# UBC-AWP/vision-sam3-yolo-lameless

Hardware: AMD Instinct MI355X
Metric: frames/sec (whole node) for YOLO+SAM3+DINOv3 feature extraction, 1080p clips (higher is better)
Workload: dtype f16; 1 GPU; BASELINE cfg#5, dense schedule: fused per-frame path on a synthetic 5 s @ 30 fps 1080p clip (150 unique BGR frames resident in HBM): YOLOv8-l detect (letterbox 384x640, NMS, scale_boxes; f16 plan) -> SAM (Hiera-B+ image encoder + FPN at 1024x1024, box-prompted mask decoder, 1080p mask + statistics + contour features) + DINOv3 ViT-L/16 embed (224x224) on EVERY frame; per-frame records packed, gathe; parallelism=one clip per GPU, 1 GPU(s), one gather per step, streams=7

## Files before the change

### vision-sam3-yolo-lameless_amd/csrc/nms.hip

```cpp
#include "common.h"

namespace {

constexpr int MAX_A = 16384;

__global__ __launch_bounds__(256) void nms_filter_kernel(const float* __restrict__ pred, int n, int A, int nc,
                                                         float conf, unsigned long long* __restrict__ keys,
                                                         int* __restrict__ counts) {
  const int64_t total = (int64_t)n * A;
  const int row_len = 4 + nc;
  for (int64_t i = (int64_t)blockIdx.x * blockDim.x + threadIdx.x; i < total; i += (int64_t)gridDim.x * blockDim.x) {
    const int img = (int)(i / A);
    const int a = (int)(i - (int64_t)img * A);
    const float* row = pred + i * row_len + 4;
    float best = row[0];
    for (int c = 1; c < nc; ++c) {
      const float v = row[c];
      best = v > best ? v : best;
    }
    if (best > conf) {
      const int slot = atomicAdd(&counts[img], 1);
      const unsigned long long key =
          ((unsigned long long)__float_as_uint(best) << 32) | (unsigned long long)(0xFFFFFFFFu - (unsigned)a);
      keys[(int64_t)img * A + slot] = key;
    }
  }
}

struct Box {
  float x1, y1, x2, y2, area;
};

__device__ __forceinline__ bool iou_gt(const Box& a, const Box& b, double thr) {
  const float xx1 = a.x1 > b.x1 ? a.x1 : b.x1;
  const float yy1 = a.y1 > b.y1 ? a.y1 : b.y1;
  const float xx2 = a.x2 < b.x2 ? a.x2 : b.x2;
  const float yy2 = a.y2 < b.y2 ? a.y2 : b.y2;
  float w = xx2 - xx1;
  w = w > 0.f ? w : 0.f;
  float h = yy2 - yy1;
  h = h > 0.f ? h : 0.f;
  const float inter = w * h;
  const float ovr = inter / (a.area + b.area - inter);
  return (double)ovr > thr;
}

__device__ __forceinline__ void bitonic_sort_desc(unsigned long long* keys, int npow2) {
  const int tid = threadIdx.x;
  for (int k = 2; k <= npow2; k <<= 1) {
    for (int j = k >> 1; j > 0; j >>= 1) {
      for (int i = tid; i < npow2; i += 1024) {
        const int ixj = i ^ j;
        if (ixj > i) {
          const unsigned long long a = keys[i], b = keys[ixj];
          const bool desc = (i & k) == 0;
          if (desc ? (a < b) : (a > b)) {
            keys[i] = b;
            keys[ixj] = a;
          }
        }
      }
      __syncthreads();
    }
  }
}

template <class Emit>
__device__ __forceinline__ int greedy_blocks(const float* __restrict__ SB, int count, double iou, int max_keep, unsigned char* supp,
                                             Box* kept, Emit emit) {
  __shared__ int s_nk;
  __shared__ int s_total;
  __shared__ int s_kept_idx[64];
  const int tid = threadIdx.x;
  const int lane = tid & 63;
  if (tid == 0) s_total = 0;
  __syncthreads();
  const int nblk = (count + 63) / 64;
// ... 159 lines not shown
  int mine = 0;
  for (int i = tid; i < npow2; i += 1024) {
    const bool v = i < n && (valid == nullptr || valid[i] != 0);
    keys[i] = v ? (((unsigned long long)score_order_key(scores[i]) << 32) | (unsigned long long)(0xFFFFFFFFu - (unsigned)i)) : 0ull;
    supp[i] = 0;
    mine += v ? 1 : 0;
    if (i < n) keep_out[i] = -1;
  }
#pragma unroll
  for (int o = 32; o > 0; o >>= 1) mine += __shfl_xor(mine, o, 64);
  if ((tid & 63) == 0 && mine) atomicAdd(&s_count, mine);
  __syncthreads();
  const int count = s_count;
  bitonic_sort_desc(keys, npow2);

  for (int i = tid; i < count; i += 1024) {
    const unsigned a = 0xFFFFFFFFu - (unsigned)(keys[i] & 0xFFFFFFFFull);
    const float* r = boxes + (int64_t)a * ldb;
    sbox[i * 5 + 0] = r[0];
    sbox[i * 5 + 1] = r[1];
    sbox[i * 5 + 2] = r[2];
    sbox[i * 5 + 3] = r[3];
    sbox[i * 5 + 4] = (r[2] - r[0]) * (r[3] - r[1]);
  }
  __syncthreads();

  const int total = greedy_blocks(sbox, count, iou, count, supp, kept, [&](int, int i, int o) {
    keep_out[o] = (int)(0xFFFFFFFFu - (unsigned)(keys[i] & 0xFFFFFFFFull));
  });
  if (tid == 0) count_out[0] = total;
}

}

extern "C" int64_t lmx_nms_workspace_bytes(int n, int A) {
  if (n <= 0 || A <= 0) return 0;
  return 256 + ((int64_t)n * 4 + 255) / 256 * 256 + (int64_t)n * A * 8 + (int64_t)n * A * 5 * 4;
}

extern "C" int lmx_k_nms(const float* pred, int n, int A, int nc, float conf, double iou, int max_det, float max_wh,
                         float* boxes, float* scores, int32_t* cls, int32_t* src, int32_t* counts, void* workspace,
                         lmx_stream_t stream) {
  LMX_REQUIRE(pred && boxes && scores && cls && src && counts && workspace, "lmx_k_nms: null pointer");
  LMX_REQUIRE(n > 0 && A > 0 && A <= MAX_A && nc > 0 && max_det > 0, "lmx_k_nms: n=%d A=%d (<=%d) nc=%d max_det=%d", n,
              A, MAX_A, nc, max_det);
  LMX_REQUIRE((((uintptr_t)workspace) & 255) == 0, "lmx_k_nms: workspace must be 256-byte aligned");
  hipStream_t st = reinterpret_cast<hipStream_t>(stream);
  char* ws = reinterpret_cast<char*>(workspace);
  int* cand_counts = reinterpret_cast<int*>(ws);
  const int64_t cnt_bytes = ((int64_t)n * 4 + 255) / 256 * 256;
  unsigned long long* keys = reinterpret_cast<unsigned long long*>(ws + cnt_bytes);
  float* sbox = reinterpret_cast<float*>(ws + cnt_bytes + (int64_t)n * A * 8);
  LMX_HIP(hipMemsetAsync(cand_counts, 0, (size_t)n * 4, st));
  int64_t g = ((int64_t)n * A + 255) / 256;
  if (g > 2048) g = 2048;
  hipLaunchKernelGGL(nms_filter_kernel, dim3((unsigned)g), dim3(256), 0, st, pred, n, A, nc, conf, keys, cand_counts);
  int rc = lmx_launch_check("nms_filter_kernel");
  if (rc) return rc;
  int npow2 = 64;
  while (npow2 < A) npow2 <<= 1;
  const size_t smem = (size_t)npow2 * 9 + 64 * sizeof(Box);
  int dev;
  LMX_TRY(lmx_stream_device(st, &dev));
  LMX_TRY(lmx_allow_lds(reinterpret_cast<const void*>(&nms_greedy_kernel), (int)((size_t)MAX_A * 9 + 64 * sizeof(Box)), dev));
  hipLaunchKernelGGL(nms_greedy_kernel, dim3(n), dim3(1024), smem, st, pred, A, nc, iou, max_det, max_wh, keys, cand_counts,
                     sbox, boxes, scores, cls, src, counts);
  return lmx_launch_check("nms_greedy_kernel");
}

extern "C" int lmx_k_nms_boxes(const float* boxes, int64_t ldb, const float* scores, const uint8_t* valid, int n, double iou,
                               int32_t* keep_out, int32_t* count_out, void* workspace, lmx_stream_t stream) {
  LMX_REQUIRE(boxes && scores && keep_out && count_out && workspace, "lmx_k_nms_boxes: null pointer");
  LMX_REQUIRE(n > 0 && n <= MAX_A && ldb >= 4, "lmx_k_nms_boxes: n=%d (1..%d) ldb=%lld", n, MAX_A, (long long)ldb);
  LMX_REQUIRE((((uintptr_t)workspace) & 15) == 0, "lmx_k_nms_boxes: workspace must be 16-byte aligned");
  int npow2 = 64;
  while (npow2 < n) npow2 <<= 1;
  const size_t smem = (size_t)npow2 * 9 + 64 * sizeof(Box);
  hipStream_t st = reinterpret_cast<hipStream_t>(stream);
  int dev;
  LMX_TRY(lmx_stream_device(st, &dev));
  LMX_TRY(lmx_allow_lds(reinterpret_cast<const void*>(&nms_boxes_kernel), (int)((size_t)MAX_A * 9 + 64 * sizeof(Box)), dev));
  hipLaunchKernelGGL(nms_boxes_kernel, dim3(1), dim3(1024), smem, st, boxes, ldb, scores, valid, n, iou, reinterpret_cast<float*>(workspace),
                     keep_out, count_out);
  return lmx_launch_check("nms_boxes_kernel");
}
```

### vision-sam3-yolo-lameless_amd/csrc/pre.hip

```cpp
#include "common.h"

namespace {

constexpr int PRECISION_BITS = 32 - 8 - 2;

__device__ __forceinline__ uint8_t clip8(int v) {
  v >>= PRECISION_BITS;
  return (uint8_t)(v < 0 ? 0 : (v > 255 ? 255 : v));
}

constexpr int RESIZE_H_MAX_ROW = 16384;
__global__ __launch_bounds__(256) void pil_resize_h_kernel(const uint8_t* __restrict__ src, uint8_t* __restrict__ dst,
                                                           int n, int sh, int sw, int dw,
                                                           const int32_t* __restrict__ bounds,
                                                           const int32_t* __restrict__ kk, int ksize, int swap_rb) {
  __shared__ __attribute__((aligned(16))) uint8_t rowbuf[RESIZE_H_MAX_ROW];
  const int rowb = sw * 3;
  for (int64_t row = blockIdx.x; row < (int64_t)n * sh; row += gridDim.x) {
    const uint8_t* srow = src + row * rowb;
    const int mis = (int)(reinterpret_cast<uintptr_t>(srow) & 15);
    const int head = mis ? 16 - mis : 0;
    for (int i = threadIdx.x; i < head && i < rowb; i += blockDim.x) rowbuf[i] = srow[i];
    const int nvec = (rowb - head) > 0 ? (rowb - head) / 16 : 0;
    for (int v = threadIdx.x; v < nvec; v += blockDim.x) {
      const u32x4 x = *reinterpret_cast<const u32x4*>(srow + head + v * 16);
      uint8_t* d = rowbuf + head + v * 16;
      if ((head & 3) == 0) {
        reinterpret_cast<unsigned*>(d)[0] = x[0];
        reinterpret_cast<unsigned*>(d)[1] = x[1];
        reinterpret_cast<unsigned*>(d)[2] = x[2];
        reinterpret_cast<unsigned*>(d)[3] = x[3];
      } else {
#pragma unroll
        for (int e = 0; e < 16; ++e) d[e] = (uint8_t)(x[e >> 2] >> (8 * (e & 3)));
      }
    }
    for (int i = head + nvec * 16 + threadIdx.x; i < rowb; i += blockDim.x) rowbuf[i] = srow[i];
    __syncthreads();
    uint8_t* drow = dst + row * dw * 3;
    for (int xo = threadIdx.x; xo < dw; xo += blockDim.x) {
      const int xmin = bounds[2 * xo], cnt = bounds[2 * xo + 1];
      const int32_t* k = kk + (int64_t)xo * ksize;
      const uint8_t* s = rowbuf + xmin * 3;
      int a0 = 1 << (PRECISION_BITS - 1), a1 = a0, a2 = a0;
      for (int x = 0; x < cnt; ++x) {
        const int c = k[x];
        a0 += (int)s[3 * x + 0] * c;
        a1 += (int)s[3 * x + 1] * c;
        a2 += (int)s[3 * x + 2] * c;
      }
      uint8_t* d = drow + xo * 3;
      if (swap_rb) {
        d[0] = clip8(a2);
        d[1] = clip8(a1);
        d[2] = clip8(a0);
      } else {
        d[0] = clip8(a0);
        d[1] = clip8(a1);
        d[2] = clip8(a2);
      }
    }
    __syncthreads();
  }
}

__global__ __launch_bounds__(256) void pil_resize_v_kernel(const uint8_t* __restrict__ src, uint8_t* __restrict__ dst,
                                                           int n, int sh, int dh, int w,
                                                           const int32_t* __restrict__ bounds,
                                                           const int32_t* __restrict__ kk, int ksize) {
  const int rowb = w * 3;
  const int64_t total = (int64_t)n * dh * rowb;
  for (int64_t i = (int64_t)blockIdx.x * blockDim.x + threadIdx.x; i < total; i += (int64_t)gridDim.x * blockDim.x) {
    const int xb = (int)(i % rowb);
    const int64_t r = i / rowb;
    const int yo = (int)(r % dh);
    const int img = (int)(r / dh);
    const int ymin = bounds[2 * yo], cnt = bounds[2 * yo + 1];
    const int32_t* k = kk + (int64_t)yo * ksize;
    const uint8_t* s = src + ((int64_t)img * sh + ymin) * rowb + xb;
    int a = 1 << (PRECISION_BITS - 1);
    for (int y = 0; y < cnt; ++y) a += (int)s[(int64_t)y * rowb] * k[y];
    dst[i] = clip8(a);
  }
}

__global__ __launch_bounds__(256) void pil_resize_v4_kernel(const uint8_t* __restrict__ src, uint8_t* __restrict__ dst, int n, int sh,
                                                            int dh, int w, const int32_t* __restrict__ bounds,
                                                            const int32_t* __restrict__ kk, int ksize) {
  const int rowb = w * 3, roww = rowb / 4;
  const int64_t total = (int64_t)n * dh * roww;
  for (int64_t i = (int64_t)blockIdx.x * blockDim.x + threadIdx.x; i < total; i += (int64_t)gridDim.x * blockDim.x) {
    const int xw = (int)(i % roww);
    const int64_t r = i / roww;
    const int yo = (int)(r % dh);
    const int img = (int)(r / dh);
    const int ymin = bounds[2 * yo], cnt = bounds[2 * yo + 1];
    const int32_t* k = kk + (int64_t)yo * ksize;
    const uint8_t* s = src + ((int64_t)img * sh + ymin) * rowb + xw * 4;
    int a0 = 1 << (PRECISION_BITS - 1), a1 = a0, a2 = a0, a3 = a0;
    for (int y = 0; y < cnt; ++y) {
      const unsigned v = *reinterpret_cast<const unsigned*>(s + (int64_t)y * rowb);
      const int c = k[y];
      a0 += (int)(v & 255u) * c;
      a1 += (int)((v >> 8) & 255u) * c;
      a2 += (int)((v >> 16) & 255u) * c;
      a3 += (int)(v >> 24) * c;
    }
    *reinterpret_cast<unsigned*>(dst + r * rowb + xw * 4) =
        (unsigned)clip8(a0) | ((unsigned)clip8(a1) << 8) | ((unsigned)clip8(a2) << 16) | ((unsigned)clip8(a3) << 24);
  }
}

__global__ __launch_bounds__(256) void patchify_norm_kernel(const uint8_t* __restrict__ img, half_t* __restrict__ out,
                                                            int n, int ih, int iw, int top, int left, int gh, int gw,
                                                            int P, int64_t ldo, const float* __restrict__ lut) {
  const int ch = gh * P, cw = gw * P;
  const int64_t total = (int64_t)n * ch * cw;
  for (int64_t i = (int64_t)blockIdx.x * blockDim.x + threadIdx.x; i < total; i += (int64_t)gridDim.x * blockDim.x) {
    const int x = (int)(i % cw);
    const int64_t r = i / cw;
    const int y = (int)(r % ch);
    const int b = (int)(r / ch);
    const uint8_t* s = img + (((int64_t)b * ih + top + y) * iw + left + x) * 3;
    const int py = y / P, ky = y - py * P, px = x / P, kx = x - px * P;
    half_t* d = out + (((int64_t)b * gh + py) * gw + px) * ldo + (ky * P + kx) * 3;
#pragma unroll
    for (int c = 0; c < 3; ++c) d[c] = (half_t)lut[c * 256 + s[c]];
  }
}

constexpr int FR_ROWS = 8;
constexpr int FR_COLS = 256;
constexpr int FR_MAX_LDS = 65536;

__global__ __launch_bounds__(FR_COLS) void float_resize_patchify_kernel(
    const uint8_t* __restrict__ src, half_t* __restrict__ out, int sh, int sw, int gh, int gw, int P, int64_t ldo,
    const int32_t* __restrict__ bh, const float* __restrict__ kh, int ksh, const int32_t* __restrict__ bv,
    const float* __restrict__ kv, int ksv, int seg_cols, float rescale, float m0, float m1, float m2, float s0, float s1,
    float s2, int swap_rb) {
  extern __shared__ __attribute__((aligned(16))) float seg[];
  const int tid = threadIdx.x;
  const int dh = gh * P, dw = gw * P;
  const int img = blockIdx.z;
  const int x0 = blockIdx.x * FR_COLS, xo = x0 + tid;
  const int y0 = blockIdx.y * FR_ROWS;
  const bool live = xo < dw;
  const int xl = (x0 + FR_COLS < dw ? x0 + FR_COLS : dw) - 1;
  int c_lo = bh[2 * x0];
  c_lo = c_lo < 0 ? 0 : (c_lo > sw ? sw : c_lo);
  int c_hi = bh[2 * xl] + bh[2 * xl + 1];
  c_hi = c_hi > sw ? sw : c_hi;
  if (c_hi > c_lo + seg_cols) c_hi = c_lo + seg_cols;
  if (c_hi < c_lo) c_hi = c_lo;
  int xmin = 0, xcnt = 0;
  if (live) {
    xmin = bh[2 * xo];
    xcnt = bh[2 * xo + 1];
    if (xmin < c_lo) xmin = c_lo;
    if (xcnt > ksh) xcnt = ksh;
    if (xcnt > c_hi - xmin) xcnt = c_hi - xmin;
    if (xcnt < 0) xcnt = 0;
  }
// ... 44 lines not shown
        f[3] = (float)(x[q] >> 24) * rescale;
        d[q] = f;
      }
    }
    for (int i = head + nvec * 16 + tid; i < nbytes; i += FR_COLS) s[i] = (float)srow[i] * rescale;
    __syncthreads();
    float h0 = 0.f, h1 = 0.f, h2 = 0.f;
    const float* p = s + (xmin - c_lo) * 3;
    for (int j = 0; j < xcnt; ++j) {
      const float w = kx[j];
      h0 = __builtin_fmaf(p[3 * j + 0], w, h0);
      h1 = __builtin_fmaf(p[3 * j + 1], w, h1);
      h2 = __builtin_fmaf(p[3 * j + 2], w, h2);
    }
#pragma unroll
    for (int r = 0; r < FR_ROWS; ++r) {
      if (y >= ymin[r] && y < ymin[r] + ycnt[r]) {
        const float w = kv[(int64_t)(y0 + r) * ksv + (y - ymin[r])];
        acc[r][0] = __builtin_fmaf(h0, w, acc[r][0]);
        acc[r][1] = __builtin_fmaf(h1, w, acc[r][1]);
        acc[r][2] = __builtin_fmaf(h2, w, acc[r][2]);
      }
    }
    __syncthreads();
  }
  if (!live) return;
  const int px = xo / P, kxp = xo - px * P;
#pragma unroll
  for (int r = 0; r < FR_ROWS; ++r) {
    const int yo = y0 + r;
    if (yo >= dh) break;
    const int py = yo / P, ky = yo - py * P;
    half_t* d = out + (((int64_t)img * gh + py) * gw + px) * ldo + (ky * P + kxp) * 3;
    d[0] = (half_t)(((swap_rb ? acc[r][2] : acc[r][0]) - m0) / s0);
    d[1] = (half_t)((acc[r][1] - m1) / s1);
    d[2] = (half_t)(((swap_rb ? acc[r][0] : acc[r][2]) - m2) / s2);
  }
}

inline int grid_for(int64_t total) {
  int64_t g = (total + 255) / 256;
  if (g > 256 * 8) g = 256 * 8;
  if (g < 1) g = 1;
  return (int)g;
}

}

extern "C" int lmx_k_pil_resize_h(const uint8_t* src, uint8_t* dst, int n, int sh, int sw, int dw, const int32_t* bounds,
                                  const int32_t* kk, int ksize, int swap_rb, lmx_stream_t stream) {
  LMX_REQUIRE(src && dst && bounds && kk, "lmx_k_pil_resize_h: null pointer");
  LMX_REQUIRE(n > 0 && sh > 0 && sw > 0 && dw > 0 && ksize > 0, "lmx_k_pil_resize_h: shape");
  LMX_REQUIRE(sw * 3 <= RESIZE_H_MAX_ROW, "lmx_k_pil_resize_h: source rows wider than %d pixels are not staged", RESIZE_H_MAX_ROW / 3);
  int64_t rows = (int64_t)n * sh;
  hipLaunchKernelGGL(pil_resize_h_kernel, dim3((unsigned)(rows < 256 * 16 ? rows : 256 * 16)), dim3(256), 0,
                     reinterpret_cast<hipStream_t>(stream), src, dst, n, sh, sw, dw, bounds, kk, ksize, swap_rb);
  return lmx_launch_check("pil_resize_h_kernel");
}

extern "C" int lmx_k_pil_resize_v(const uint8_t* src, uint8_t* dst, int n, int sh, int dh, int w, const int32_t* bounds,
                                  const int32_t* kk, int ksize, lmx_stream_t stream) {
  LMX_REQUIRE(src && dst && bounds && kk, "lmx_k_pil_resize_v: null pointer");
  LMX_REQUIRE(n > 0 && sh > 0 && dh > 0 && w > 0 && ksize > 0, "lmx_k_pil_resize_v: shape");
  if ((w * 3) % 4 == 0 && (((uintptr_t)src | (uintptr_t)dst) & 3) == 0) {
    hipLaunchKernelGGL(pil_resize_v4_kernel, dim3(grid_for((int64_t)n * dh * (w * 3 / 4))), dim3(256), 0,
                       reinterpret_cast<hipStream_t>(stream), src, dst, n, sh, dh, w, bounds, kk, ksize);
    return lmx_launch_check("pil_resize_v4_kernel");
  }
  hipLaunchKernelGGL(pil_resize_v_kernel, dim3(grid_for((int64_t)n * dh * w * 3)), dim3(256), 0,
                     reinterpret_cast<hipStream_t>(stream), src, dst, n, sh, dh, w, bounds, kk, ksize);
  return lmx_launch_check("pil_resize_v_kernel");
}

extern "C" int lmx_k_float_resize_patchify(const uint8_t* src, void* out, int n, int sh, int sw, int gh, int gw, int P,
                                           int64_t ldo, const int32_t* bounds_h, const float* kk_h, int ksize_h,
                                           const int32_t* bounds_v, const float* kk_v, int ksize_v, int seg_cols,
                                           float rescale, const float* mean_std, int swap_rb, lmx_stream_t stream) {
  LMX_REQUIRE(src && out && bounds_h && kk_h && bounds_v && kk_v && mean_std, "lmx_k_float_resize_patchify: null pointer");
  LMX_REQUIRE(n > 0 && n <= 65535 && sh > 0 && sw > 0 && gh > 0 && gw > 0 && P > 0 && ksize_h > 0 && ksize_v > 0,
              "lmx_k_float_resize_patchify: shape");
  LMX_REQUIRE(ldo >= (int64_t)P * P * 3, "lmx_k_float_resize_patchify: ldo %lld < P*P*3", (long long)ldo);
  LMX_REQUIRE((int64_t)gh * P <= 65535 * (int64_t)FR_ROWS && (int64_t)gw * P <= (1 << 20), "lmx_k_float_resize_patchify: output size");
  LMX_REQUIRE(seg_cols > 0 && seg_cols <= sw, "lmx_k_float_resize_patchify: seg_cols %d outside 1..%d", seg_cols, sw);
  const int64_t lds = ((int64_t)seg_cols * 3 + 4) * (int64_t)sizeof(float);
  LMX_REQUIRE(lds <= FR_MAX_LDS, "lmx_k_float_resize_patchify: a tile of %d output columns reads %d source columns; more than %d are not staged",
              FR_COLS, seg_cols, (FR_MAX_LDS / 4 - 4) / 3);
  LMX_REQUIRE(mean_std[3] != 0.f && mean_std[4] != 0.f && mean_std[5] != 0.f, "lmx_k_float_resize_patchify: zero std");
  const dim3 grid((unsigned)((gw * P + FR_COLS - 1) / FR_COLS), (unsigned)((gh * P + FR_ROWS - 1) / FR_ROWS), (unsigned)n);
  hipLaunchKernelGGL(float_resize_patchify_kernel, grid, dim3(FR_COLS), (size_t)lds, reinterpret_cast<hipStream_t>(stream), src,
                     reinterpret_cast<half_t*>(out), sh, sw, gh, gw, P, ldo, bounds_h, kk_h, ksize_h, bounds_v, kk_v, ksize_v,
                     seg_cols, rescale, mean_std[0], mean_std[1], mean_std[2], mean_std[3], mean_std[4], mean_std[5], swap_rb);
  return lmx_launch_check("float_resize_patchify_kernel");
}

extern "C" int lmx_k_patchify_norm(const uint8_t* img, void* out, int n, int ih, int iw, int top, int left, int gh,
                                   int gw, int P, int64_t ldo, const float* lut, lmx_stream_t stream) {
  LMX_REQUIRE(img && out && lut, "lmx_k_patchify_norm: null pointer");
  LMX_REQUIRE(n > 0 && gh > 0 && gw > 0 && P > 0 && ldo >= (int64_t)P * P * 3, "lmx_k_patchify_norm: shape");
  LMX_REQUIRE(top >= 0 && left >= 0 && top + gh * P <= ih && left + gw * P <= iw,
              "lmx_k_patchify_norm: crop (%d,%d)+(%d,%d) outside %dx%d", top, left, gh * P, gw * P, ih, iw);
  hipLaunchKernelGGL(patchify_norm_kernel, dim3(grid_for((int64_t)n * gh * P * gw * P)), dim3(256), 0,
                     reinterpret_cast<hipStream_t>(stream), img, reinterpret_cast<half_t*>(out), n, ih, iw, top, left, gh,
                     gw, P, ldo, lut);
  return lmx_launch_check("patchify_norm_kernel");
}
```

### vision-sam3-yolo-lameless_amd/csrc/sam.hip

```cpp
#include "common.h"
#include "hiera_bands.h"

namespace {

inline int grid_for(int64_t total, int block = 256) {
  int64_t g = (total + block - 1) / block;
  if (g > 256 * 8) g = 256 * 8;
  if (g < 1) g = 1;
  return (int)g;
}

template <int KW_T>
__global__ __launch_bounds__(256) void im2col_u8_kernel(const uint8_t* __restrict__ img, const float* __restrict__ lut,
                                                        half_t* __restrict__ out, int n, int rh, int rw, int OH, int OW, int KH,
                                                        int KW_rt, int stride, int pad, int64_t ldo) {
  __shared__ float lut_s[768];
  for (int i = threadIdx.x; i < 768; i += blockDim.x) lut_s[i] = lut[i];
  __syncthreads();
  const int KW = KW_T > 0 ? KW_T : KW_rt;
  const int chunks = (int)(ldo / 8);
  const int K = KH * KW * 3;
  const int64_t total = (int64_t)n * OH * OW * chunks;
  for (int64_t i = (int64_t)blockIdx.x * blockDim.x + threadIdx.x; i < total; i += (int64_t)gridDim.x * blockDim.x) {
    const int ck = (int)(i % chunks);
    const int64_t tok = i / chunks;
    const int ox = (int)(tok % OW);
    const int64_t r = tok / OW;
    const int oy = (int)(r % OH);
    const int b = (int)(r / OH);
    const uint8_t* ib = img + (int64_t)b * rh * rw * 3;
    const int y0 = oy * stride - pad, x0 = ox * stride - pad;
    half8_t v;
#pragma unroll
    for (int e = 0; e < 8; ++e) {
      const int k = ck * 8 + e;
      float val = 0.f;
      if (k < K) {
        const int tap = k / 3, c = k - tap * 3;
        const int ky = tap / KW, kx = tap - ky * KW;
        const int y = y0 + ky, x = x0 + kx;
        if ((unsigned)y < (unsigned)rh && (unsigned)x < (unsigned)rw) val = lut_s[c * 256 + ib[(y * rw + x) * 3 + c]];
      }
      v[e] = (half_t)val;
    }
    *reinterpret_cast<half8_t*>(out + tok * ldo + ck * 8) = v;
  }
}

template <typename T, int VEC>
__global__ __launch_bounds__(256) void maxpool2_kernel(const T* __restrict__ src, int64_t lds, T* __restrict__ dst, int64_t ldd,
                                                       int n, int H, int W, int C) {
  typedef T vec_t __attribute__((ext_vector_type(VEC)));
  const int cc = C / VEC;
  const int Ho = H / 2, Wo = W / 2;
  const int64_t total = (int64_t)n * Ho * Wo * cc;
  for (int64_t i = (int64_t)blockIdx.x * blockDim.x + threadIdx.x; i < total; i += (int64_t)gridDim.x * blockDim.x) {
    const int c = (int)(i % cc) * VEC;
    const int64_t p = i / cc;
    const int x = (int)(p % Wo);
    const int64_t r = p / Wo;
    const int y = (int)(r % Ho);
    const int b = (int)(r / Ho);
// ... 216 lines not shown
  const int64_t total = rows * wb;
  const bool fast = (w & 7) == 0 && ((reinterpret_cast<uintptr_t>(src) & 7) == 0);
  for (int64_t i = (int64_t)blockIdx.x * blockDim.x + threadIdx.x; i < total; i += (int64_t)gridDim.x * blockDim.x) {
    const int64_t r = i / wb;
    const int c = (int)(i - r * wb);
    const uint8_t* sp = src + r * w + (int64_t)c * 8;
    unsigned long long x = 0;
    if (fast) {
      x = *reinterpret_cast<const unsigned long long*>(sp);
    } else {
      for (int e = 0; e < 8; ++e)
        if (c * 8 + e < w) x |= (unsigned long long)sp[e] << (8 * e);
    }
    x = (x | (x >> 1) | (x >> 2) | (x >> 3) | (x >> 4) | (x >> 5) | (x >> 6) | (x >> 7)) & 0x0101010101010101ull;
    dst[i] = (uint8_t)((x * 0x8040201008040201ull) >> 56);
  }
}

__global__ __launch_bounds__(256) void prompt_box_kernel(const float* __restrict__ boxes, int64_t ldb, float* __restrict__ sparse,
                                                        int n, double sx, double sy, float S, const float* __restrict__ gauss,
                                                        const float* __restrict__ corner, int F) {
  const int i = blockIdx.x * blockDim.x + threadIdx.x;
  if (i >= n * 2 * F) return;
  const int j = i % F, k = (i / F) & 1, b = i / (2 * F);
  const float* bx = boxes + (int64_t)b * ldb + 2 * k;
  const float px = (float)((double)bx[0] * sx) + 0.5f, py = (float)((double)bx[1] * sy) + 0.5f;
  const float cx = 2.f * (px / S) - 1.f, cy = 2.f * (py / S) - 1.f;
  const float ang = 6.283185307179586f * (cx * gauss[j] + cy * gauss[F + j]);
  float* o = sparse + ((int64_t)b * 2 + k) * 2 * F;
  o[j] = sinf(ang) + corner[k * 2 * F + j];
  o[F + j] = cosf(ang) + corner[k * 2 * F + F + j];
}

__global__ void mask_stats_init_kernel(long long* stats, int n) {
  const int i = blockIdx.x * blockDim.x + threadIdx.x;
  if (i >= n * 8) return;
  const int f = i & 7;
  stats[i] = (f == 3 || f == 4) ? 0x7fffffffll : ((f == 5 || f == 6) ? -1ll : 0ll);
}

}

extern "C" int lmx_k_im2col_u8(const uint8_t* img, const float* lut, void* out, int n, int rh, int rw, int IH, int IW, int KH,
                               int KW, int stride, int pad, int64_t ldo, lmx_stream_t stream) {
  LMX_REQUIRE(img && lut && out, "lmx_k_im2col_u8: null pointer");
  LMX_REQUIRE(n > 0 && rh > 0 && rw > 0 && rh <= IH && rw <= IW && KH > 0 && KW > 0 && stride > 0 && pad >= 0,
              "lmx_k_im2col_u8: geometry");
  LMX_REQUIRE(ldo % 8 == 0 && ldo >= (int64_t)KH * KW * 3 && aligned16(out), "lmx_k_im2col_u8: ldo/alignment");
  const int OH = (IH + 2 * pad - KH) / stride + 1, OW = (IW + 2 * pad - KW) / stride + 1;
  LMX_REQUIRE((int64_t)rh * rw * 3 < 0x7fffffffll, "lmx_k_im2col_u8: frame too large");
  const dim3 grid(grid_for((int64_t)n * OH * OW * (ldo / 8)));
  hipStream_t st = reinterpret_cast<hipStream_t>(stream);
  half_t* o16 = reinterpret_cast<half_t*>(out);
  if (KW == 7)
    hipLaunchKernelGGL((im2col_u8_kernel<7>), grid, dim3(256), 0, st, img, lut, o16, n, rh, rw, OH, OW, KH, KW, stride, pad, ldo);
  else if (KW == 16)
    hipLaunchKernelGGL((im2col_u8_kernel<16>), grid, dim3(256), 0, st, img, lut, o16, n, rh, rw, OH, OW, KH, KW, stride, pad, ldo);
  else
    hipLaunchKernelGGL((im2col_u8_kernel<0>), grid, dim3(256), 0, st, img, lut, o16, n, rh, rw, OH, OW, KH, KW, stride, pad, ldo);
  return lmx_launch_check("im2col_u8_kernel");
}

extern "C" int lmx_k_maxpool2(const void* src, int64_t lds, void* dst, int64_t ldd, int dtype, int n, int H, int W, int C,
                              lmx_stream_t stream) {
  LMX_REQUIRE(src && dst, "lmx_k_maxpool2: null pointer");
  LMX_REQUIRE(n > 0 && H > 0 && W > 0 && H % 2 == 0 && W % 2 == 0 && C > 0 && lds >= C && ldd >= C, "lmx_k_maxpool2: shape");
  hipStream_t st = reinterpret_cast<hipStream_t>(stream);
  if (dtype == LMX_F16) {
    LMX_REQUIRE(C % 8 == 0 && lds % 8 == 0 && ldd % 8 == 0 && aligned16(src) && aligned16(dst), "lmx_k_maxpool2: f16 alignment");
    hipLaunchKernelGGL((maxpool2_kernel<half_t, 8>), dim3(grid_for((int64_t)n * (H / 2) * (W / 2) * (C / 8))), dim3(256), 0, st,
                       reinterpret_cast<const half_t*>(src), lds, reinterpret_cast<half_t*>(dst), ldd, n, H, W, C);
  } else if (dtype == LMX_F32) {
    LMX_REQUIRE(C % 4 == 0 && lds % 4 == 0 && ldd % 4 == 0 && aligned16(src) && aligned16(dst), "lmx_k_maxpool2: f32 alignment");
    hipLaunchKernelGGL((maxpool2_kernel<float, 4>), dim3(grid_for((int64_t)n * (H / 2) * (W / 2) * (C / 4))), dim3(256), 0, st,
                       reinterpret_cast<const float*>(src), lds, reinterpret_cast<float*>(dst), ldd, n, H, W, C);
  } else {
    LMX_REQUIRE(false, "lmx_k_maxpool2: dtype %d", dtype);
  }
  return lmx_launch_check("maxpool2_kernel");
}

extern "C" int lmx_k_cast_f32_f16(const float* src, int64_t lds, void* dst, int64_t ldd, int64_t rows, int cols,
                                  lmx_stream_t stream) {
  LMX_REQUIRE(src && dst, "lmx_k_cast_f32_f16: null pointer");
  LMX_REQUIRE(rows > 0 && cols > 0 && cols % 4 == 0 && lds % 4 == 0 && ldd % 4 == 0 && lds >= cols && ldd >= cols,
              "lmx_k_cast_f32_f16: shape");
  LMX_REQUIRE(aligned16(src) && ((((uintptr_t)dst) & 7) == 0), "lmx_k_cast_f32_f16: alignment");
  hipLaunchKernelGGL(cast_kernel, dim3(grid_for(rows * (cols / 4))), dim3(256), 0, reinterpret_cast<hipStream_t>(stream), src, lds,
                     reinterpret_cast<half_t*>(dst), ldd, rows, cols);
  return lmx_launch_check("cast_kernel");
}

extern "C" int lmx_h_hiera_band(const int* window, const int* q_stride, int n_blocks, int grid, int nh, int nw, int* band) {
  LMX_REQUIRE(window && q_stride && band, "lmx_h_hiera_band: null pointer");
  LMX_REQUIRE(n_blocks > 0 && grid > 0 && grid <= (1 << 20) && nh > 0 && nw > 0 && nh <= 4 * grid && nw <= 4 * grid,
              "lmx_h_hiera_band: n_blocks=%d grid=%d nh=%d nw=%d", n_blocks, grid, nh, nw);
  *band = 0;
  if (nw < 4 * grid) return LMX_OK;
  int64_t unit = 1, scale = 1;
  int first_global = -1;
  for (int i = 0; i < n_blocks; ++i) {
    LMX_REQUIRE(window[i] >= 0 && (q_stride[i] == 0 || q_stride[i] == 1 || q_stride[i] == 2), "lmx_h_hiera_band: block %d: window=%d q_stride=%d",
                i, window[i], q_stride[i]);
    if (window[i] == 0) {
      first_global = i;
      break;
    }
    const int64_t pieces[2] = {window[i] * scale, q_stride[i] == 2 ? 2 * scale : scale};
    for (int64_t p : pieces) {
// ... 129 lines not shown
```

### vision-sam3-yolo-lameless_amd/csrc/yolo.hip

```cpp
#include "common.h"

namespace {

inline int grid_for(int64_t total, int block = 256) {
  int64_t g = (total + block - 1) / block;
  if (g > 256 * 8) g = 256 * 8;
  if (g < 1) g = 1;
  return (int)g;
}

__global__ __launch_bounds__(256) void letterbox_kernel(const uint8_t* __restrict__ src, uint8_t* __restrict__ dst, int n,
                                                        int sh, int sw, int rh, int rw, int top, int left, int oh, int ow,
                                                        const int* __restrict__ xofs, const short* __restrict__ ialpha,
                                                        const int* __restrict__ yofs, const short* __restrict__ ibeta,
                                                        int swap_rb, int identity) {
  const int64_t total = (int64_t)n * oh * ow;
  for (int64_t i = (int64_t)blockIdx.x * blockDim.x + threadIdx.x; i < total; i += (int64_t)gridDim.x * blockDim.x) {
    const int ox = (int)(i % ow);
    const int64_t r = i / ow;
    const int oy = (int)(r % oh);
    const int img = (int)(r / oh);
    uint8_t* d = dst + i * 3;
    const int dy = oy - top, dx = ox - left;
    if (dy < 0 || dy >= rh || dx < 0 || dx >= rw) {
// ... 128 lines not shown
    const int b = (int)(r / Ho);
    *reinterpret_cast<half8_t*>(dst + p * ldd + c) =
        *reinterpret_cast<const half8_t*>(src + (((int64_t)b * H + (y >> 1)) * W + (x >> 1)) * lds + c);
  }
}

__global__ __launch_bounds__(256) void detect_decode_kernel(const float* __restrict__ head, float* __restrict__ pred, int n,
                                                            int H, int W, int nc, int ch, float stride, int a_off,
                                                            int A) {
  const int64_t total = (int64_t)n * H * W * 4;
  for (int64_t i0 = (int64_t)blockIdx.x * blockDim.x; i0 < total; i0 += (int64_t)gridDim.x * blockDim.x) {
    const int64_t i = i0 + threadIdx.x;
    const bool live = i < total;
    const int side = (int)(i & 3);
    const int64_t cell = live ? (i >> 2) : 0;
    const int x = (int)(cell % W);
    const int64_t r = cell / W;
    const int y = (int)(r % H);
    const int b = (int)(r / H);
    const float* hrow = head + cell * ch;
    float l[16];
    float mx = -INFINITY;
#pragma unroll
    for (int k = 0; k < 4; ++k) {
      const f32x4 v = *reinterpret_cast<const f32x4*>(hrow + side * 16 + k * 4);
#pragma unroll
      for (int e = 0; e < 4; ++e) {
        l[k * 4 + e] = v[e];
        mx = fmaxf(mx, v[e]);
      }
    }
    float se = 0.f;
#pragma unroll
    for (int k = 0; k < 16; ++k) {
      l[k] = expf(l[k] - mx);
      se += l[k];
    }
    float dist = 0.f;
#pragma unroll
    for (int k = 0; k < 16; ++k) dist += (l[k] / se) * (float)k;
    const int base = threadIdx.x & ~3;
    const float dl = __shfl(dist, (base & 63) + 0, 64), dt = __shfl(dist, (base & 63) + 1, 64);
    const float dr = __shfl(dist, (base & 63) + 2, 64), db = __shfl(dist, (base & 63) + 3, 64);
    if (!live) continue;
    float* prow = pred + ((int64_t)b * A + a_off + (int64_t)y * W + x) * (4 + nc);
    if (side == 0) {
      const float ax = (float)x + 0.5f, ay = (float)y + 0.5f;
      const float x1 = ax - dl, y1 = ay - dt, x2 = ax + dr, y2 = ay + db;
      prow[0] = ((x1 + x2) / 2.f) * stride;
      prow[1] = ((y1 + y2) / 2.f) * stride;
      prow[2] = (x2 - x1) * stride;
      prow[3] = (y2 - y1) * stride;
    }
    for (int c = side; c < nc; c += 4) {
      const float v = hrow[64 + c];
      prow[4 + c] = 1.0f / (1.0f + expf(-v));
    }
  }
}

__global__ __launch_bounds__(256) void scale_boxes_kernel(float* __restrict__ boxes, int total, float padx, float pady,
                                                          float gain, float w, float h) {
  const int i = blockIdx.x * blockDim.x + threadIdx.x;
  if (i >= total) return;
  float* b = boxes + (int64_t)i * 4;
  float x1 = (b[0] - padx) / gain, y1 = (b[1] - pady) / gain, x2 = (b[2] - padx) / gain, y2 = (b[3] - pady) / gain;
  b[0] = fminf(fmaxf(x1, 0.f), w);
  b[1] = fminf(fmaxf(y1, 0.f), h);
  b[2] = fminf(fmaxf(x2, 0.f), w);
  b[3] = fminf(fmaxf(y2, 0.f), h);
}

struct PoseLevels {
  const float* raw[3];
  int h[3], w[3], off[3];
  float stride[3];
};
__global__ __launch_bounds__(256) void pose_gather_kernel(const PoseLevels L, int64_t ldk, const int* __restrict__ src,
                                                          const int* __restrict__ counts, int n, int max_det, int K, int ndim,
                                                          float padx, float pady, float gain, float fw, float fh,
                                                          float* __restrict__ out) {
  const int64_t total = (int64_t)n * max_det * K;
  for (int64_t i = (int64_t)blockIdx.x * blockDim.x + threadIdx.x; i < total; i += (int64_t)gridDim.x * blockDim.x) {
    const int k = (int)(i % K);
    const int64_t r = i / K;
    const int j = (int)(r % max_det);
    const int b = (int)(r / max_det);
    float* o = out + i * ndim;
    if (j >= counts[b]) {
      for (int e = 0; e < ndim; ++e) o[e] = 0.f;
      continue;
    }
    const int a = src[(int64_t)b * max_det + j];
    const int l = a >= L.off[2] ? 2 : (a >= L.off[1] ? 1 : 0);
    const int local = a - L.off[l];
    const int y = local / L.w[l], x = local - y * L.w[l];
    const float* v = L.raw[l] + (((int64_t)b * L.h[l] + y) * L.w[l] + x) * ldk + k * ndim;
    const float X = (v[0] * 2.0f + (float)x) * L.stride[l];
    const float Y = (v[1] * 2.0f + (float)y) * L.stride[l];
    o[0] = fminf(fmaxf((X - padx) / gain, 0.f), fw);
    o[1] = fminf(fmaxf((Y - pady) / gain, 0.f), fh);
    if (ndim == 3) o[2] = 1.0f / (1.0f + expf(-v[2]));
  }
}

}

extern "C" int lmx_k_pose_gather(const float* raw0, const float* raw1, const float* raw2, int64_t ldk, const int32_t* hw,
                                 const float* strides, const int32_t* src, const int32_t* counts, int n, int max_det, int K,
                                 int ndim, float padx, float pady, float gain, float w, float h, float* out,
// ... 90 lines not shown
```

Before: 788.8 frames/s.

## Vectorize NMS filter, PIL resize, SAM patch im2col and YOLO sigmoid writes

```diff
diff --git a/vision-sam3-yolo-lameless_amd/csrc/nms.hip b/vision-sam3-yolo-lameless_amd/csrc/nms.hip
--- a/vision-sam3-yolo-lameless_amd/csrc/nms.hip
+++ b/vision-sam3-yolo-lameless_amd/csrc/nms.hip
@@ -4,25 +4,57 @@
 
 constexpr int MAX_A = 16384;
 
+template <bool VEC>
 __global__ __launch_bounds__(256) void nms_filter_kernel(const float* __restrict__ pred, int n, int A, int nc,
                                                          float conf, unsigned long long* __restrict__ keys,
                                                          int* __restrict__ counts) {
   const int64_t total = (int64_t)n * A;
   const int row_len = 4 + nc;
-  for (int64_t i = (int64_t)blockIdx.x * blockDim.x + threadIdx.x; i < total; i += (int64_t)gridDim.x * blockDim.x) {
-    const int img = (int)(i / A);
-    const int a = (int)(i - (int64_t)img * A);
-    const float* row = pred + i * row_len + 4;
-    float best = row[0];
-    for (int c = 1; c < nc; ++c) {
-      const float v = row[c];
-      best = v > best ? v : best;
-    }
-    if (best > conf) {
-      const int slot = atomicAdd(&counts[img], 1);
-      const unsigned long long key =
-          ((unsigned long long)__float_as_uint(best) << 32) | (unsigned long long)(0xFFFFFFFFu - (unsigned)a);
-      keys[(int64_t)img * A + slot] = key;
+  const int pieces = VEC ? row_len / 4 : row_len;
+  const int L = pieces < 64 ? pieces : 64;
+  const int rpw = 64 / L;
+  const int lane = threadIdx.x & 63;
+  const int r = lane / L, q = lane - r * L;
+  const int64_t wave = (int64_t)blockIdx.x * (blockDim.x >> 6) + (threadIdx.x >> 6);
+  const int64_t step = (int64_t)gridDim.x * (blockDim.x >> 6) * rpw;
+  for (int64_t base = wave * rpw; base < total; base += step) {
+    const int64_t i = base + r;
+    const bool live = r < rpw && i < total;
+    const int img = live ? (int)(i / A) : 0;
+    float best = -__builtin_inff();
+    if (live) {
+      const float* row = pred + i * row_len;
+      if (VEC) {
+        for (int u = q > 0 ? q : L; u < pieces; u += L) {
+          const f32x4 v = *reinterpret_cast<const f32x4*>(row + 4 * u);
+#pragma unroll
+          for (int e = 0; e < 4; ++e) best = v[e] > best ? v[e] : best;
+        }
+      } else {
+        for (int u = q; u < pieces; u += L) {
+          const float v = row[u];
+          best = (u >= 4 && v > best) ? v : best;
+        }
+      }
+    }
+    for (int off = 1; off < L; off <<= 1) {
+      const float o = __shfl_down(best, off, 64);
+      best = (q + off < L && o > best) ? o : best;
+    }
+    const bool pass = live && q == 0 && best > conf;
+    const unsigned long long key =
+        ((unsigned long long)__float_as_uint(best) << 32) | (unsigned long long)(0xFFFFFFFFu - (unsigned)(i - (int64_t)img * A));
+    unsigned long long todo = __ballot(pass);
+    while (todo) {
+      const int lead = __ffsll((long long)todo) - 1;
+      const int img_l = __shfl(img, lead, 64);
+      const bool mine = pass && img == img_l;
+      const unsigned long long m = __ballot(mine);
+      int slot = 0;
+      if (lane == lead) slot = atomicAdd(&counts[img_l], __popcll(m));
+      slot = __shfl(slot, lead, 64) + __popcll(m & ((1ull << lane) - 1ull));
+      if (mine) keys[(int64_t)img * A + slot] = key;
+      todo &= ~m;
     }
   }
 }
@@ -288,9 +320,15 @@
   unsigned long long* keys = reinterpret_cast<unsigned long long*>(ws + cnt_bytes);
   float* sbox = reinterpret_cast<float*>(ws + cnt_bytes + (int64_t)n * A * 8);
   LMX_HIP(hipMemsetAsync(cand_counts, 0, (size_t)n * 4, st));
-  int64_t g = ((int64_t)n * A + 255) / 256;
+  const bool vec = (4 + nc) % 4 == 0 && (((uintptr_t)pred) & 15) == 0;
+  const int pieces = vec ? (4 + nc) / 4 : 4 + nc;
+  const int rows_wg = 4 * (64 / (pieces < 64 ? pieces : 64));
+  int64_t g = ((int64_t)n * A + rows_wg - 1) / rows_wg;
   if (g > 2048) g = 2048;
-  hipLaunchKernelGGL(nms_filter_kernel, dim3((unsigned)g), dim3(256), 0, st, pred, n, A, nc, conf, keys, cand_counts);
+  if (vec)
+    hipLaunchKernelGGL(nms_filter_kernel<true>, dim3((unsigned)g), dim3(256), 0, st, pred, n, A, nc, conf, keys, cand_counts);
+  else
+    hipLaunchKernelGGL(nms_filter_kernel<false>, dim3((unsigned)g), dim3(256), 0, st, pred, n, A, nc, conf, keys, cand_counts);
   int rc = lmx_launch_check("nms_filter_kernel");
   if (rc) return rc;
   int npow2 = 64;
diff --git a/vision-sam3-yolo-lameless_amd/csrc/pre.hip b/vision-sam3-yolo-lameless_amd/csrc/pre.hip
--- a/vision-sam3-yolo-lameless_amd/csrc/pre.hip
+++ b/vision-sam3-yolo-lameless_amd/csrc/pre.hip
@@ -5,59 +5,86 @@
 constexpr int PRECISION_BITS = 32 - 8 - 2;
 
 __device__ __forceinline__ uint8_t clip8(int v) {
-  v >>= PRECISION_BITS;
-  return (uint8_t)(v < 0 ? 0 : (v > 255 ? 255 : v));
-}
+  const int top = (256 << PRECISION_BITS) - 1;
+  v = v < 0 ? 0 : (v > top ? top : v);
+  return (uint8_t)((unsigned)v >> PRECISION_BITS);
+}
+
+__device__ __forceinline__ int tap(unsigned byte, int coef) { return __mul24((int)byte, coef); }
 
 constexpr int RESIZE_H_MAX_ROW = 16384;
+constexpr int RESIZE_H_LDS = 2 * RESIZE_H_MAX_ROW;
+constexpr int RESIZE_H_ROWS = 4;
+
+inline int resize_h_group(int rowb) {
+  int r = (RESIZE_H_LDS - 16) / rowb;
+  r = r > 8 ? 8 : r;
+  return r >= RESIZE_H_ROWS ? r / RESIZE_H_ROWS * RESIZE_H_ROWS : r;
+}
+
 __global__ __launch_bounds__(256) void pil_resize_h_kernel(const uint8_t* __restrict__ src, uint8_t* __restrict__ dst,
-                                                           int n, int sh, int sw, int dw,
+                                                           int n, int sh, int sw, int dw, int group,
                                                            const int32_t* __restrict__ bounds,
                                                            const int32_t* __restrict__ kk, int ksize, int swap_rb) {
-  __shared__ __attribute__((aligned(16))) uint8_t rowbuf[RESIZE_H_MAX_ROW];
+  __shared__ __attribute__((aligned(16))) uint8_t buf[RESIZE_H_LDS];
   const int rowb = sw * 3;
-  for (int64_t row = blockIdx.x; row < (int64_t)n * sh; row += gridDim.x) {
-    const uint8_t* srow = src + row * rowb;
-    const int mis = (int)(reinterpret_cast<uintptr_t>(srow) & 15);
-    const int head = mis ? 16 - mis : 0;
-    for (int i = threadIdx.x; i < head && i < rowb; i += blockDim.x) rowbuf[i] = srow[i];
-    const int nvec = (rowb - head) > 0 ? (rowb - head) / 16 : 0;
-    for (int v = threadIdx.x; v < nvec; v += blockDim.x) {
-      const u32x4 x = *reinterpret_cast<const u32x4*>(srow + head + v * 16);
-      uint8_t* d = rowbuf + head + v * 16;
-      if ((head & 3) == 0) {
-        reinterpret_cast<unsigned*>(d)[0] = x[0];
-        reinterpret_cast<unsigned*>(d)[1] = x[1];
-        reinterpret_cast<unsigned*>(d)[2] = x[2];
-        reinterpret_cast<unsigned*>(d)[3] = x[3];
-      } else {
-#pragma unroll
-        for (int e = 0; e < 16; ++e) d[e] = (uint8_t)(x[e >> 2] >> (8 * (e & 3)));
-      }
-    }
-    for (int i = head + nvec * 16 + threadIdx.x; i < rowb; i += blockDim.x) rowbuf[i] = srow[i];
+  const int64_t rows = (int64_t)n * sh;
+  const int dwq = (dw + 3) & ~3;
+  for (int64_t row0 = (int64_t)blockIdx.x * group; row0 < rows; row0 += (int64_t)gridDim.x * group) {
+    const int nr = rows - row0 < group ? (int)(rows - row0) : group;
+    const uint8_t* s0 = src + row0 * rowb;
+    const int span = nr * rowb;
+    const int mis = (int)(reinterpret_cast<uintptr_t>(s0) & 15);
+    int head = mis ? 16 - mis : 0;
+    head = head > span ? span : head;
+    for (int i = threadIdx.x; i < head; i += blockDim.x) buf[mis + i] = s0[i];
+    const int nvec = (span - head) / 16;
+    for (int v = threadIdx.x; v < nvec; v += blockDim.x)
+      *reinterpret_cast<u32x4*>(buf + mis + head + v * 16) = *reinterpret_cast<const u32x4*>(s0 + head + v * 16);
+    for (int i = head + nvec * 16 + threadIdx.x; i < span; i += blockDim.x) buf[mis + i] = s0[i];
     __syncthreads();
-    uint8_t* drow = dst + row * dw * 3;
-    for (int xo = threadIdx.x; xo < dw; xo += blockDim.x) {
+    const int ntask = dwq * ((nr + RESIZE_H_ROWS - 1) / RESIZE_H_ROWS);
+    for (int t0 = 0; t0 < ntask; t0 += blockDim.x) {
+      const int t = t0 + threadIdx.x;
+      const int rg = t / dwq, xq = t - rg * dwq;
+      const int r0 = rg * RESIZE_H_ROWS;
+      const bool live = t < ntask && xq < dw;
+      const int xo = xq < dw ? xq : dw - 1;
+      int rb[RESIZE_H_ROWS];
+#pragma unroll
+      for (int r = 0; r < RESIZE_H_ROWS; ++r) rb[r] = mis + (r0 + r < nr ? r0 + r : nr - 1) * rowb;
       const int xmin = bounds[2 * xo], cnt = bounds[2 * xo + 1];
       const int32_t* k = kk + (int64_t)xo * ksize;
-      const uint8_t* s = rowbuf + xmin * 3;
-      int a0 = 1 << (PRECISION_BITS - 1), a1 = a0, a2 = a0;
+      int a[RESIZE_H_ROWS][3];
+#pragma unroll
+      for (int r = 0; r < RESIZE_H_ROWS; ++r) a[r][0] = a[r][1] = a[r][2] = 1 << (PRECISION_BITS - 1);
       for (int x = 0; x < cnt; ++x) {
         const int c = k[x];
-        a0 += (int)s[3 * x + 0] * c;
-        a1 += (int)s[3 * x + 1] * c;
-        a2 += (int)s[3 * x + 2] * c;
-      }
-      uint8_t* d = drow + xo * 3;
-      if (swap_rb) {
-        d[0] = clip8(a2);
-        d[1] = clip8(a1);
-        d[2] = clip8(a0);
-      } else {
-        d[0] = clip8(a0);
-        d[1] = clip8(a1);
-        d[2] = clip8(a2);
+        const int off = (xmin + x) * 3;
+#pragma unroll
+        for (int r = 0; r < RESIZE_H_ROWS; ++r) {
+          const uint8_t* s = buf + rb[r] + off;
+          a[r][0] += tap(s[0], c);
+          a[r][1] += tap(s[1], c);
+          a[r][2] += tap(s[2], c);
+        }
+      }
+      const int j = xq & 3;
+      const bool quad = xq - j + 4 <= dw;
+#pragma unroll
+      for (int r = 0; r < RESIZE_H_ROWS; ++r) {
+        const unsigned b0 = clip8(swap_rb ? a[r][2] : a[r][0]), b1 = clip8(a[r][1]), b2 = clip8(swap_rb ? a[r][0] : a[r][2]);
+        const unsigned px = b0 | (b1 << 8) | (b2 << 16);
+        const unsigned nx = __shfl_down(px, 1, 64);
+        if (!live || r0 + r >= nr) continue;
+        uint8_t* d = dst + (row0 + r0 + r) * dw * 3 + xq * 3;
+        if (quad && ((reinterpret_cast<uintptr_t>(d) - 3 * j) & 3) == 0) {
+          if (j < 3) *reinterpret_cast<unsigned*>(d - 3 * j + 4 * j) = (px >> (8 * j)) | (nx << (24 - 8 * j));
+        } else {
+          d[0] = (uint8_t)b0;
+          d[1] = (uint8_t)b1;
+          d[2] = (uint8_t)b2;
+        }
       }
     }
     __syncthreads();
@@ -79,15 +106,17 @@
     const int32_t* k = kk + (int64_t)yo * ksize;
     const uint8_t* s = src + ((int64_t)img * sh + ymin) * rowb + xb;
     int a = 1 << (PRECISION_BITS - 1);
-    for (int y = 0; y < cnt; ++y) a += (int)s[(int64_t)y * rowb] * k[y];
+    for (int y = 0; y < cnt; ++y) a += tap(s[(int64_t)y * rowb], k[y]);
     dst[i] = clip8(a);
   }
 }
 
-__global__ __launch_bounds__(256) void pil_resize_v4_kernel(const uint8_t* __restrict__ src, uint8_t* __restrict__ dst, int n, int sh,
+template <int DW>
+__global__ __launch_bounds__(256) void pil_resize_vw_kernel(const uint8_t* __restrict__ src, uint8_t* __restrict__ dst, int n, int sh,
                                                             int dh, int w, const int32_t* __restrict__ bounds,
                                                             const int32_t* __restrict__ kk, int ksize) {
-  const int rowb = w * 3, roww = rowb / 4;
+  typedef unsigned vec_t __attribute__((ext_vector_type(DW)));
+  const int rowb = w * 3, roww = (rowb + 4 * DW - 1) / (4 * DW);
   const int64_t total = (int64_t)n * dh * roww;
   for (int64_t i = (int64_t)blockIdx.x * blockDim.x + threadIdx.x; i < total; i += (int64_t)gridDim.x * blockDim.x) {
     const int xw = (int)(i % roww);
@@ -96,18 +125,35 @@
     const int img = (int)(r / dh);
     const int ymin = bounds[2 * yo], cnt = bounds[2 * yo + 1];
     const int32_t* k = kk + (int64_t)yo * ksize;
-    const uint8_t* s = src + ((int64_t)img * sh + ymin) * rowb + xw * 4;
-    int a0 = 1 << (PRECISION_BITS - 1), a1 = a0, a2 = a0, a3 = a0;
+    const int xb = xw * (4 * DW) + 4 * DW <= rowb ? xw * (4 * DW) : rowb - 4 * DW;
+    const uint8_t* s = src + ((int64_t)img * sh + ymin) * rowb + xb;
+    int a[4 * DW];
+#pragma unroll
+    for (int e = 0; e < 4 * DW; ++e) a[e] = 1 << (PRECISION_BITS - 1);
     for (int y = 0; y < cnt; ++y) {
-      const unsigned v = *reinterpret_cast<const unsigned*>(s + (int64_t)y * rowb);
+      vec_t v;
+      if (DW == 4)
+        v = *reinterpret_cast<const vec_t*>(s + (int64_t)y * rowb);
+      else
+        __builtin_memcpy(&v, s + (int64_t)y * rowb, sizeof(v));
       const int c = k[y];
-      a0 += (int)(v & 255u) * c;
-      a1 += (int)((v >> 8) & 255u) * c;
-      a2 += (int)((v >> 16) & 255u) * c;
-      a3 += (int)(v >> 24) * c;
-    }
-    *reinterpret_cast<unsigned*>(dst + r * rowb + xw * 4) =
-        (unsigned)clip8(a0) | ((unsigned)clip8(a1) << 8) | ((unsigned)clip8(a2) << 16) | ((unsigned)clip8(a3) << 24);
+#pragma unroll
+      for (int q = 0; q < DW; ++q) {
+        a[4 * q + 0] += tap(v[q] & 255u, c);
+        a[4 * q + 1] += tap((v[q] >> 8) & 255u, c);
+        a[4 * q + 2] += tap((v[q] >> 16) & 255u, c);
+        a[4 * q + 3] += tap(v[q] >> 24, c);
+      }
+    }
+    vec_t o;
+#pragma unroll
+    for (int q = 0; q < DW; ++q)
+      o[q] = (unsigned)clip8(a[4 * q]) | ((unsigned)clip8(a[4 * q + 1]) << 8) | ((unsigned)clip8(a[4 * q + 2]) << 16) |
+             ((unsigned)clip8(a[4 * q + 3]) << 24);
+    if (DW == 4)
+      *reinterpret_cast<vec_t*>(dst + r * rowb + xb) = o;
+    else
+      __builtin_memcpy(dst + r * rowb + xb, &o, sizeof(o));
   }
 }
 
@@ -258,9 +304,10 @@
   LMX_REQUIRE(src && dst && bounds && kk, "lmx_k_pil_resize_h: null pointer");
   LMX_REQUIRE(n > 0 && sh > 0 && sw > 0 && dw > 0 && ksize > 0, "lmx_k_pil_resize_h: shape");
   LMX_REQUIRE(sw * 3 <= RESIZE_H_MAX_ROW, "lmx_k_pil_resize_h: source rows wider than %d pixels are not staged", RESIZE_H_MAX_ROW / 3);
-  int64_t rows = (int64_t)n * sh;
-  hipLaunchKernelGGL(pil_resize_h_kernel, dim3((unsigned)(rows < 256 * 16 ? rows : 256 * 16)), dim3(256), 0,
-                     reinterpret_cast<hipStream_t>(stream), src, dst, n, sh, sw, dw, bounds, kk, ksize, swap_rb);
+  const int group = resize_h_group(sw * 3);
+  const int64_t groups = ((int64_t)n * sh + group - 1) / group;
+  hipLaunchKernelGGL(pil_resize_h_kernel, dim3((unsigned)(groups < 256 * 16 ? groups : 256 * 16)), dim3(256), 0,
+                     reinterpret_cast<hipStream_t>(stream), src, dst, n, sh, sw, dw, group, bounds, kk, ksize, swap_rb);
   return lmx_launch_check("pil_resize_h_kernel");
 }
 
@@ -268,10 +315,16 @@
                                   const int32_t* kk, int ksize, lmx_stream_t stream) {
   LMX_REQUIRE(src && dst && bounds && kk, "lmx_k_pil_resize_v: null pointer");
   LMX_REQUIRE(n > 0 && sh > 0 && dh > 0 && w > 0 && ksize > 0, "lmx_k_pil_resize_v: shape");
-  if ((w * 3) % 4 == 0 && (((uintptr_t)src | (uintptr_t)dst) & 3) == 0) {
-    hipLaunchKernelGGL(pil_resize_v4_kernel, dim3(grid_for((int64_t)n * dh * (w * 3 / 4))), dim3(256), 0,
+  const uintptr_t al = (uintptr_t)src | (uintptr_t)dst | (uintptr_t)(w * 3);
+  if ((al & 15) == 0) {
+    hipLaunchKernelGGL(pil_resize_vw_kernel<4>, dim3(grid_for((int64_t)n * dh * (w * 3 / 16))), dim3(256), 0,
                        reinterpret_cast<hipStream_t>(stream), src, dst, n, sh, dh, w, bounds, kk, ksize);
-    return lmx_launch_check("pil_resize_v4_kernel");
+    return lmx_launch_check("pil_resize_vw_kernel<4>");
+  }
+  if (w * 3 >= 4) {
+    hipLaunchKernelGGL(pil_resize_vw_kernel<1>, dim3(grid_for((int64_t)n * dh * ((w * 3 + 3) / 4))), dim3(256), 0,
+                       reinterpret_cast<hipStream_t>(stream), src, dst, n, sh, dh, w, bounds, kk, ksize);
+    return lmx_launch_check("pil_resize_vw_kernel<1>");
   }
   hipLaunchKernelGGL(pil_resize_v_kernel, dim3(grid_for((int64_t)n * dh * w * 3)), dim3(256), 0,
                      reinterpret_cast<hipStream_t>(stream), src, dst, n, sh, dh, w, bounds, kk, ksize);
diff --git a/vision-sam3-yolo-lameless_amd/csrc/sam.hip b/vision-sam3-yolo-lameless_amd/csrc/sam.hip
--- a/vision-sam3-yolo-lameless_amd/csrc/sam.hip
+++ b/vision-sam3-yolo-lameless_amd/csrc/sam.hip
@@ -8,6 +8,103 @@
   if (g > 256 * 8) g = 256 * 8;
   if (g < 1) g = 1;
   return (int)g;
+}
+
+constexpr int P7_T = 64;
+constexpr int P7_ROW = (4 * P7_T + 3) * 3;
+constexpr int P7_NDW = (P7_ROW + 3 + 3) / 4 + 1;
+constexpr int P7_LOADS = (7 * P7_NDW + 255) / 256;
+__global__ __launch_bounds__(256) void im2col_p7_kernel(const uint8_t* __restrict__ img, const float* __restrict__ lut,
+                                                        half_t* __restrict__ out, int n, int rh, int rw, int OH, int OW, int64_t ldo) {
+  __shared__ half_t lut_s[768];
+  __shared__ half_t st[7 * P7_ROW];
+  for (int i = threadIdx.x; i < 768; i += blockDim.x) lut_s[i] = (half_t)lut[i];
+  __syncthreads();
+  const int tid = threadIdx.x;
+  const int chunks = (int)(ldo / 8);
+  const int tpp = 256 / chunks;
+  const int tl = tid / chunks, ck = tid - tl * chunks;
+  int offs[8];
+  unsigned zeros = 0u;
+#pragma unroll
+  for (int e = 0; e < 8; ++e) {
+    const int k = ck * 8 + e, ky = k / 21;
+    offs[e] = k < 147 ? ky * P7_ROW + (k - ky * 21) : 0;
+    zeros |= k < 147 ? 0u : 1u << e;
+  }
+  const int runs = (OW + P7_T - 1) / P7_T;
+  const int64_t jobs = (int64_t)n * OH * runs;
+  for (int64_t job = blockIdx.x; job < jobs; job += gridDim.x) {
+    const int run = (int)(job % runs);
+    const int64_t r = job / runs;
+    const int oy = (int)(r % OH);
+    const int b = (int)(r / OH);
+    const int ox0 = run * P7_T;
+    const int tc = OW - ox0 < P7_T ? OW - ox0 : P7_T;
+    const int x_lo = ox0 * 4 - 3;
+    const int nst = (4 * tc + 3) * 3;
+    const int xa = x_lo > 0 ? x_lo : 0;
+    const int xb = x_lo + 4 * tc + 3 < rw ? x_lo + 4 * tc + 3 : rw;
+    const int lo = (xa - x_lo) * 3, len = (xb - xa) * 3;
+    const uint8_t* ib = img + (int64_t)b * rh * rw * 3;
+    for (int ky = 0; ky < 7; ++ky) {
+      const bool in = (unsigned)(oy * 4 - 3 + ky) < (unsigned)rh && len > 0;
+      half_t* srow = st + ky * P7_ROW;
+      for (int i = tid; i < (in ? lo : nst); i += blockDim.x) srow[i] = (half_t)0.f;
+      for (int i = (in ? lo + len : nst) + tid; i < nst; i += blockDim.x) srow[i] = (half_t)0.f;
+    }
+    unsigned v[P7_LOADS], units = 0u;
+    int j0[P7_LOADS], at[P7_LOADS];
+#pragma unroll
+    for (int it = 0; it < P7_LOADS; ++it) {
+      const int u = tid + it * 256;
+      const int ky = u / P7_NDW, d = u - ky * P7_NDW;
+      const int y = oy * 4 - 3 + ky;
+      v[it] = 0u;
+      j0[it] = at[it] = 0;
+      if (ky < 7 && (unsigned)y < (unsigned)rh && len > 0) {
+        const uint8_t* g = ib + (y * rw + xa) * 3;
+        const int mis = (int)(reinterpret_cast<uintptr_t>(g) & 3);
+        const int j = d * 4 - mis;
+        if (j < len) {
+          units |= 1u << it;
+          j0[it] = j;
+          at[it] = ky * P7_ROW + lo + j;
+          if (j >= 0 && j + 4 <= len) {
+            v[it] = *reinterpret_cast<const unsigned*>(g + j);
+          } else {
+#pragma unroll
+            for (int e = 0; e < 4; ++e)
+              if (j + e >= 0 && j + e < len) v[it] |= (unsigned)g[j + e] << (8 * e);
+          }
+        }
+      }
+    }
+#pragma unroll
+    for (int it = 0; it < P7_LOADS; ++it) {
+      if (!((units >> it) & 1u)) continue;
+      int c = (j0[it] + 3) % 3;
+#pragma unroll
+      for (int e = 0; e < 4; ++e) {
+        if (j0[it] + e >= 0 && j0[it] + e < len) st[at[it] + e] = lut_s[c * 256 + ((v[it] >> (8 * e)) & 255u)];
+        c = c == 2 ? 0 : c + 1;
+      }
+    }
+    __syncthreads();
+    half_t* orow = out + (((int64_t)b * OH + oy) * OW + ox0) * ldo + ck * 8;
+    if (tl < tpp) {
+      for (int t = tl; t < tc; t += tpp) {
+        half8_t o;
+#pragma unroll
+        for (int e = 0; e < 8; ++e) {
+          const half_t val = st[offs[e] + t * 12];
+          o[e] = (zeros >> e) & 1u ? (half_t)0.f : val;
+        }
+        *reinterpret_cast<half8_t*>(orow + (int64_t)t * ldo) = o;
+      }
+    }
+    __syncthreads();
+  }
 }
 
 template <int KW_T>
@@ -330,9 +427,12 @@
   const dim3 grid(grid_for((int64_t)n * OH * OW * (ldo / 8)));
   hipStream_t st = reinterpret_cast<hipStream_t>(stream);
   half_t* o16 = reinterpret_cast<half_t*>(out);
-  if (KW == 7)
-    hipLaunchKernelGGL((im2col_u8_kernel<7>), grid, dim3(256), 0, st, img, lut, o16, n, rh, rw, OH, OW, KH, KW, stride, pad, ldo);
-  else if (KW == 16)
+  if (KH == 7 && KW == 7 && stride == 4 && pad == 3 && ldo <= 8 * 256) {
+    const int64_t jobs = (int64_t)n * OH * ((OW + P7_T - 1) / P7_T);
+    hipLaunchKernelGGL(im2col_p7_kernel, dim3(grid_for(jobs * 256)), dim3(256), 0, st, img, lut, o16, n, rh, rw, OH, OW, ldo);
+    return lmx_launch_check("im2col_p7_kernel");
+  }
+  if (KW == 16)
     hipLaunchKernelGGL((im2col_u8_kernel<16>), grid, dim3(256), 0, st, img, lut, o16, n, rh, rw, OH, OW, KH, KW, stride, pad, ldo);
   else
     hipLaunchKernelGGL((im2col_u8_kernel<0>), grid, dim3(256), 0, st, img, lut, o16, n, rh, rw, OH, OW, KH, KW, stride, pad, ldo);
diff --git a/vision-sam3-yolo-lameless_amd/csrc/yolo.hip b/vision-sam3-yolo-lameless_amd/csrc/yolo.hip
--- a/vision-sam3-yolo-lameless_amd/csrc/yolo.hip
+++ b/vision-sam3-yolo-lameless_amd/csrc/yolo.hip
@@ -204,10 +204,23 @@
       prow[2] = (x2 - x1) * stride;
       prow[3] = (y2 - y1) * stride;
     }
-    for (int c = side; c < nc; c += 4) {
-      const float v = hrow[64 + c];
-      prow[4 + c] = 1.0f / (1.0f + expf(-v));
-    }
+    const float* hc = hrow + 64;
+    float* pc = prow + 4;
+    const bool al = (reinterpret_cast<uintptr_t>(pc) & 15) == 0;
+    const int nc4 = nc & ~3;
+    for (int c = side * 4; c < nc4; c += 16) {
+      const f32x4 v = *reinterpret_cast<const f32x4*>(hc + c);
+      f32x4 s;
+#pragma unroll
+      for (int e = 0; e < 4; ++e) s[e] = 1.0f / (1.0f + expf(-v[e]));
+      if (al) {
+        *reinterpret_cast<f32x4*>(pc + c) = s;
+      } else {
+#pragma unroll
+        for (int e = 0; e < 4; ++e) pc[c + e] = s[e];
+      }
+    }
+    for (int c = nc4 + side; c < nc; c += 4) pc[c] = 1.0f / (1.0f + expf(-hc[c]));
   }
 }
 
```

Measured after the change: 801.8 frames/s (median of 6 runs). 1.7% higher.
